# emreatilgan/P-Companion

Hardware: AMD Instinct MI355X
Metric: triplets/sec (Product2Vec pretrain step: gather+fwd+bwd+Adam) + P-Companion joint step under `joint` (higher is better)
Workload: dtype f32

## Files before the change

include/pcompanion_hip.h:

```cpp
#ifndef PCOMPANION_HIP_H
#define PCOMPANION_HIP_H

#include <stddef.h>
#include <stdint.h>

#ifdef __cplusplus
extern "C" {
#endif

#define PC_OK 0
#define PC_EINVAL (-1)
#define PC_ESHAPE (-2)
#define PC_EWORKSPACE (-3)
#define PC_EBATCHNORM (-4)
#define PC_ECOMM (-5)

#define PC_D 128
#define PC_H 256
#define PC_HEADS 4
#define PC_L 64
#define PC_MAX_SEG 4
#define PC_BN_SYNC_DOUBLES (PC_MAX_SEG * 2 * 256 + PC_MAX_SEG)

#define PC_ABI_VERSION 8
int pc_abi_version(void);
enum { PC_OPT_SIDE_QUEUE = 1, PC_OPT_SORTED_TABLE_GRADIENTS = 2, PC_OPT_BN_FINALIZE_SIDE = 3, PC_OPT_FUSED_LOSS = 4,
       PC_OPT_FUSED_OUT_CHAIN = 5 };
int pc_set_option(int option, int value);
int pc_get_option(int option, int* value);
int pc_release_device_state(void);
enum {
    PC_FLAG_EXP_NO_MFMA = 1, PC_FLAG_EXP_NO_SPLIT = 2, PC_FLAG_EXP_NO_LDSREAD = 4, PC_FLAG_EXP_NO_DMA = 8,
    PC_FLAG_EXP_NO_SLAB = 16, PC_FLAG_EXP_STAGGER = 32, PC_FLAG_EXP_DMA_L2 = 64, PC_FLAG_NT_TIMING = 128,
    PC_FLAG_JOINT_TIMING = 256, PC_FLAG_CHAIN_TIMING = 512, PC_FLAG_EXP_NO_BARRIER = 1024, PC_FLAG_EXP_NO_VMWAIT = 2048
};
unsigned pc_build_flags(void);

typedef struct {
    float p;
    uint64_t seed, offset;
} pc_dropout;

// ... 423 lines not shown
```

p_companion_amd/_lib.py:

```python
import ctypes
import os

_HERE = os.path.dirname(os.path.abspath(__file__))
LIB_PATH = os.path.join(_HERE, "libpcompanion_hip.so")
if os.environ.get("PC_DEV_LIB"):
    import sys as _sys
    LIB_PATH = os.path.abspath(os.environ["PC_DEV_LIB"])
    print(f"[p_companion_amd] PC_DEV_LIB: loading {LIB_PATH} instead of the in-tree library (developer A/B run)", file=_sys.stderr, flush=True)

c_f32p = ctypes.c_void_p
c_i32p = ctypes.c_void_p
PC_MAX_SEG = 4
D, H, HEADS, L = 128, 256, 4, 64

_ERR = {-1: "PC_EINVAL (null pointer / bad size)", -2: "PC_ESHAPE (unsupported dimension/alignment)",
        -3: "PC_EWORKSPACE (workspace too small)",
        -4: "PC_EBATCHNORM (a BatchNorm call group of one row in training mode)",
        -5: "PC_ECOMM (RCCL could not be loaded, or a communicator call failed)"}


class HipKernelError(RuntimeError):
    pass


# ... 33 lines not shown

_vp, _i, _sz, _f, _d, _u64, _i64 = (ctypes.c_void_p, ctypes.c_int, ctypes.c_size_t, ctypes.c_float,
                                    ctypes.c_double, ctypes.c_uint64, ctypes.c_int64)
_P = ctypes.POINTER

class AdamFused(ctypes.Structure):
    _fields_ = [("param", ctypes.c_void_p), ("grad", ctypes.c_void_p), ("exp_avg", ctypes.c_void_p), ("exp_avg_sq", ctypes.c_void_p),
                ("n", ctypes.c_size_t), ("step_count", ctypes.c_void_p), ("t", ctypes.c_int64),
                ("lr", ctypes.c_double), ("beta1", ctypes.c_double), ("beta2", ctypes.c_double), ("eps", ctypes.c_double)]


PC_OPT_SIDE_QUEUE = 1
PC_OPT_FUSED_OUT_CHAIN = 5
PC_OPT_FUSED_LOSS = 4
PC_OPT_BN_FINALIZE_SIDE = 3
PC_OPT_SORTED_TABLE_GRADIENTS = 2

SIGNATURES = {
    "pc_abi_version": (_i, []),
    "pc_build_flags": (ctypes.c_uint, []),
    "pc_set_option": (_i, [_i, _i]),
    "pc_get_option": (_i, [_i, ctypes.POINTER(ctypes.c_int)]),
    "pc_release_device_state": (_i, []),
    "pc_p2v_ffn_workspace_bytes": (_sz, [_i]),
    "pc_p2v_ffn_forward_train": (_i, [_P(P2VTensors), _vp, _vp, _i, _P(Segments), _i, _vp, _P(FfnSaved), _vp, _sz, _vp]),
    "pc_p2v_ffn_forward_eval": (_i, [_P(P2VTensors), _vp, _vp, _i, _vp, _vp, _sz, _vp]),
    "pc_p2v_ffn_backward": (_i, [_P(P2VTensors), _P(P2VTensors), _vp, _vp, _i, _P(Segments), _vp, _P(FfnSaved),
                                 _vp, _i, _vp, _sz, _vp]),
    "pc_p2v_attention_workspace_bytes": (_sz, [_i, _i]),
    "pc_p2v_attention_workspace_bytes_dim": (_sz, [_i, _i, _i]),
# ... 162 lines not shown
```

p_companion_amd/csrc/common.h:

```cpp
#pragma once
#include <hip/hip_runtime.h>
#include <stdint.h>
#include "../../include/pcompanion_hip.h"

typedef float f32x16 __attribute__((ext_vector_type(16)));
typedef float f32x4 __attribute__((ext_vector_type(4)));

#define PC_WAVE 64

#define PC_HIP_TRY(expr)                          \
    do {                                          \
        hipError_t _e = (expr);                   \
        if (_e != hipSuccess) return (int)_e;     \
    } while (0)

#define PC_TRY(expr)                 \
    do {                             \
        int _r = (expr);             \
        if (_r != 0) return _r;      \
    } while (0)

extern thread_local int pc_tls_launch_err;
#define PC_LAUNCH(...)                                                           \
    do {                                                                         \
// ... 425 lines not shown
struct TnArgs {
    const float* Z; int ldz;
    const float* A; int lda; const int32_t* gather;
    int R, No, Ni;
    SegInfo seg;
    int prologue; const float* pscale; const float* pshift;
    const float* zaux; int ldzaux;
    const float *z_mean, *z_invstd, *z_scale, *z_c1, *z_c2;
    const int32_t* z_onehot;
    float* dW; int lddw; float* db;
    int accumulate;
    float* slabs; size_t slab_floats;
};
struct TnDefer;
int launch_gemm_tn(const TnArgs& a, hipStream_t st, TnDefer* defer = nullptr);
int launch_gemm_tn_halves(const TnArgs& a, float* slabs0, float* slabs1, size_t slab_floats, hipStream_t st, TnDefer* defer);
size_t gemm_tn_workspace_floats(int R, int No, int Ni);
#define PC_TN_GROUP 10
#define PC_TN_EXTRA 2
#define PC_TN_RGROUP (PC_TN_GROUP + PC_TN_EXTRA + 4)
struct TnGroup { TnArgs a[PC_TN_GROUP]; int tiles_i[PC_TN_GROUP], nsplit[PC_TN_GROUP], rps[PC_TN_GROUP], block0[PC_TN_GROUP + 1], n; };
struct TnReduceJob { const float* slabs; int nsplit, n; float* out; int accumulate; };
#define PC_ADAM_REST (2 * (PC_TN_GROUP + PC_TN_EXTRA + 4) + 1)
struct AdamRider {
    float *p, *m, *v; const float* g; size_t n;
    int64_t* step_count; long long t; double lr, beta1, beta2; float omb1, beta2f, omb2, eps;
    int block0;
    int n_rest, rest_lo[PC_ADAM_REST], rest_hi[PC_ADAM_REST], rest_block0[PC_ADAM_REST + 1];
};
struct TnReduceGroup {
    const float* slabs[PC_TN_RGROUP]; float* dW[PC_TN_RGROUP]; float* db[PC_TN_RGROUP];
// ... 31 lines not shown
static inline void joint_fields(const pc_joint_tensors* t, float* (&out)[10]) {
    float* const f[10] = {t->itm_w, t->itm_b, t->typ_w, t->typ_b, t->dec_w, t->dec_b, t->enc_w, t->enc_b, t->comp_types, t->query_types};
    for (int i = 0; i < 10; i++) out[i] = f[i];
}
static inline bool joint_tensors_ok(const pc_joint_tensors* t, bool need_table) {
    if (!t || (need_table && !t->product_table)) return false;
    float* f[10];
    joint_fields(t, f);
    for (float* x : f)
        if (!x) return false;
    return true;
}

int pc_opt_sorted_tables();
int pc_opt_bn_finalize_side();
int pc_opt_fused_loss();
int pc_opt_fused_out_chain();
int triplet_loss_launch(const float* a, const float* p, const float* n, int batch, int k_neg, int dim, float margin,
                        float* loss, float* d_pos, float* d_neg, float* da, float* dp, float* dn, void* stream, int with_mean);
int launch_dropout(const float* x, size_t n, const pc_dropout& d, unsigned stream_id, float* y, hipStream_t st);
int launch_transpose(const float* in, int rows, int cols, float* out, hipStream_t st);
int ffn_forward_part1(const pc_p2v_tensors* p, const float* table, const int32_t* idx, int rows, const pc_segments* seg,
                      const pc_ffn_saved* sv, double* local_sums, void* ws, size_t ws_bytes, void* stream);
int ffn_forward_part2(const pc_p2v_tensors* p, int rows, const pc_segments* seg, int update_running, float* y,
                      const pc_ffn_saved* sv, const double* global_sums, void* ws, size_t ws_bytes, void* stream,
                      const TransposeBatch* ride = nullptr);
int ffn_backward_part1(const pc_p2v_tensors* p, const pc_p2v_tensors* g, const float* table, const int32_t* idx,
                       int rows, const pc_segments* seg, const float* dy, const pc_ffn_saved* sv, int with_dx,
                       int accumulate, double* local_sums, void* ws, size_t ws_bytes, void* stream, int transposed,
                       TnDefer* defer);
// ... 16 lines not shown
```

p_companion_amd/csrc/ffn.hip:

```cpp
#include "common.h"


#define BN_EPS 1e-5f
#define BN_MOMENTUM 0.1f

#define FIN_COLS 32
#define FIN_LANES 32
__device__ __forceinline__ void fold_partials(const float* p1, const float* p2, int t0, int t1, int j, int q,
                                              double (*red)[FIN_LANES][FIN_COLS], double* o1, double* o2) {
    double a = 0.0, b = 0.0, a1 = 0.0, b1 = 0.0;
    int t = t0 + q;
    for (; t + FIN_LANES < t1; t += 2 * FIN_LANES) {
        a += (double)p1[(size_t)t * PC_H + j];                b += (double)p2[(size_t)t * PC_H + j];
        a1 += (double)p1[(size_t)(t + FIN_LANES) * PC_H + j]; b1 += (double)p2[(size_t)(t + FIN_LANES) * PC_H + j];
    }
    if (t < t1) { a += (double)p1[(size_t)t * PC_H + j]; b += (double)p2[(size_t)t * PC_H + j]; }
    red[0][q][threadIdx.x] = a + a1;
    red[1][q][threadIdx.x] = b + b1;
    __syncthreads();
    if (q == 0) {
        double s1 = 0.0, s2 = 0.0;
#pragma unroll 8
        for (int i = 0; i < FIN_LANES; i++) { s1 += red[0][i][threadIdx.x]; s2 += red[1][i][threadIdx.x]; }
        *o1 = s1; *o2 = s2;
    }
    __syncthreads();
}

#define FIN4_CG 8
#define FIN4_LANES 64
#define FIN4_WAVES (FIN4_CG * FIN4_LANES / 64)
#define FIN4_BATCH 6
__device__ __forceinline__ void fold_partials_all4(const float* __restrict__ p1, const float* __restrict__ p2, const SegInfo& si,
                                                   int col0, double (*red)[2][PC_MAX_SEG][FIN_COLS], double* o1, double* o2) {
    const int cg = threadIdx.x, q = threadIdx.y;
    const int tid = q * FIN4_CG + cg, wave = tid >> 6, lane = tid & 63;
    double a[PC_MAX_SEG][4], b[PC_MAX_SEG][4];
#pragma unroll
    for (int s = 0; s < PC_MAX_SEG; s++)
#pragma unroll
        for (int c = 0; c < 4; c++) { a[s][c] = 0.0; b[s][c] = 0.0; }
    const int t_end = si.tile0[si.nseg];
    const int b1 = si.nseg > 1 ? si.tile0[1] : t_end, b2 = si.nseg > 2 ? si.tile0[2] : t_end, b3 = si.nseg > 3 ? si.tile0[3] : t_end;
    const size_t c0 = (size_t)col0 + cg * 4;
    for (int t = si.tile0[0] + q; t < t_end; t += FIN4_BATCH * FIN4_LANES) {
        float4 x[FIN4_BATCH], y[FIN4_BATCH];
#pragma unroll
        for (int u = 0; u < FIN4_BATCH; u++) {
            const int tt = t + u * FIN4_LANES;
            const int tc = tt < t_end ? tt : t;
            x[u] = *reinterpret_cast<const float4*>(p1 + (size_t)tc * PC_H + c0);
            y[u] = *reinterpret_cast<const float4*>(p2 + (size_t)tc * PC_H + c0);
        }
#pragma unroll
        for (int u = 0; u < FIN4_BATCH; u++) {
            const int tt = t + u * FIN4_LANES;
            const int sg = tt < t_end ? (tt >= b1) + (tt >= b2) + (tt >= b3) : -1;
#pragma unroll
            for (int s = 0; s < PC_MAX_SEG; s++) {
                const bool on = sg == s;
                a[s][0] += on ? (double)x[u].x : 0.0; a[s][1] += on ? (double)x[u].y : 0.0;
                a[s][2] += on ? (double)x[u].z : 0.0; a[s][3] += on ? (double)x[u].w : 0.0;
                b[s][0] += on ? (double)y[u].x : 0.0; b[s][1] += on ? (double)y[u].y : 0.0;
                b[s][2] += on ? (double)y[u].z : 0.0; b[s][3] += on ? (double)y[u].w : 0.0;
            }
        }
    }
#pragma unroll
    for (int s = 0; s < PC_MAX_SEG; s++)
#pragma unroll
        for (int c = 0; c < 4; c++) {
#pragma unroll
            for (int o = 8; o < 64; o <<= 1) { a[s][c] += __shfl_xor(a[s][c], o, 64); b[s][c] += __shfl_xor(b[s][c], o, 64); }
        }
    if (lane < FIN4_CG) {
#pragma unroll
        for (int s = 0; s < PC_MAX_SEG; s++)
#pragma unroll
            for (int c = 0; c < 4; c++) { red[wave][0][s][cg * 4 + c] = a[s][c]; red[wave][1][s][cg * 4 + c] = b[s][c]; }
    }
    __syncthreads();
    if (tid < PC_MAX_SEG * FIN_COLS) {
        const int s = tid / FIN_COLS, col = tid % FIN_COLS;
        double s1 = 0.0, s2 = 0.0;
#pragma unroll
        for (int w = 0; w < FIN4_WAVES; w++) { s1 += red[w][0][s][col]; s2 += red[w][1][s][col]; }
        *o1 = s1; *o2 = s2;
    }
}

__global__ __launch_bounds__(FIN_COLS * FIN_LANES) void bn_fold_kernel(const float* p1, const float* p2, SegInfo si,
                                                                       double* sums) {
    __shared__ double red[2][FIN_LANES][FIN_COLS];
    const int j = blockIdx.x * FIN_COLS + threadIdx.x, q = threadIdx.y;
    for (int s = 0; s < PC_MAX_SEG; s++) {
        double a = 0.0, b = 0.0;
        if (s < si.nseg) fold_partials(p1, p2, si.tile0[s], si.tile0[s + 1], j, q, red, &a, &b);
        if (q == 0) {
            sums[(2 * s) * PC_H + j] = a;
            sums[(2 * s + 1) * PC_H + j] = b;
            if (j == 0) sums[2 * PC_MAX_SEG * PC_H + s] = s < si.nseg ? (double)si.count[s] : 0.0;
        }
    }
// ... 2 lines not shown
__global__ __launch_bounds__(FIN4_CG * FIN4_LANES) void bn_finalize_fwd_kernel(
    const float* psum, const float* psq, SegInfo si, const double* gsum, const float* gamma, const float* beta,
    float* running_mean, float* running_var, int64_t* nbt, int update_running, float* mean_o, float* invstd_o,
    float* scale_o, float* shift_o, TransposeBatch ride, int tiles_x, int tiles_y) {
    __shared__ double red[FIN4_WAVES][2][PC_MAX_SEG][FIN_COLS];
    __shared__ float seg_mean[PC_MAX_SEG][FIN_COLS], seg_unb[PC_MAX_SEG][FIN_COLS];
    __shared__ int seg_live[PC_MAX_SEG][FIN_COLS];
    const int tid = threadIdx.y * FIN4_CG + threadIdx.x;
    if (blockIdx.x >= PC_H / FIN_COLS) {
        static_assert(sizeof(red) >= 32 * 33 * sizeof(float), "transpose tile");
        transpose_tile_body<FIN4_CG * FIN4_LANES>(ride, (int)blockIdx.x - PC_H / FIN_COLS, tiles_x, tiles_y,
                                                  reinterpret_cast<float(*)[33]>(&red[0][0][0][0]), tid);
        return;
    }
    double a = 0.0, b = 0.0;
    if (!gsum) fold_partials_all4(psum, psq, si, blockIdx.x * FIN_COLS, red, &a, &b);
    if (tid < PC_MAX_SEG * FIN_COLS) {
        const int s = tid / FIN_COLS, col = tid % FIN_COLS, j = blockIdx.x * FIN_COLS + col;
        double n = s < si.nseg ? (double)si.count[s] : 0.0;
        if (gsum && s < si.nseg) { a = gsum[(2 * s) * PC_H + j]; b = gsum[(2 * s + 1) * PC_H + j]; n = gsum[2 * PC_MAX_SEG * PC_H + s]; }
        int live = 0;
        if (s < si.nseg && n > 0) {
            const double m = a / n;
            double var = b / n - m * m;
            if (var < 0.0) var = 0.0;
            const float mf = (float)m, vf = (float)var;
            const float is = 1.0f / sqrtf(vf + BN_EPS);
            const float sc = gamma[j] * is;
            mean_o[s * PC_H + j] = mf;
            invstd_o[s * PC_H + j] = is;
            scale_o[s * PC_H + j] = sc;
// ... 21 lines not shown
    }
}

__global__ void bn_eval_coeff_kernel(const float* gamma, const float* beta, const float* running_mean,
                                     const float* running_var, float* scale_o, float* shift_o) {
    const int j = threadIdx.x;
    const float is = 1.0f / sqrtf(running_var[j] + BN_EPS);
    const float sc = gamma[j] * is;
    scale_o[j] = sc;
    shift_o[j] = beta[j] - running_mean[j] * sc;
}

__global__ __launch_bounds__(FIN4_CG * FIN4_LANES) void bn_finalize_bwd_kernel(
    const float* psum, const float* pdot, SegInfo si, const double* lsum, const double* gsum, const float* mean,
    const float* invstd, float* dgamma, float* dbeta, int accumulate, float* c1, float* c2) {
    __shared__ double red[FIN4_WAVES][2][PC_MAX_SEG][FIN_COLS];
    __shared__ double seg_g[PC_MAX_SEG][FIN_COLS], seg_b[PC_MAX_SEG][FIN_COLS];
    const int tid = threadIdx.y * FIN4_CG + threadIdx.x;
    double a = 0.0, b = 0.0;
    if (!lsum) fold_partials_all4(psum, pdot, si, blockIdx.x * FIN_COLS, red, &a, &b);
    if (tid < PC_MAX_SEG * FIN_COLS) {
        const int s = tid / FIN_COLS, col = tid % FIN_COLS, j = blockIdx.x * FIN_COLS + col;
        double tg = 0.0, tb = 0.0;
        if (s < si.nseg) {
            double n = si.count[s];
            if (lsum) { a = lsum[(2 * s) * PC_H + j]; b = lsum[(2 * s + 1) * PC_H + j]; }
            const double is = (double)invstd[s * PC_H + j], mu = (double)mean[s * PC_H + j];
            b = is * (b - mu * a);
            tb = a;
            tg = b;
            double ga = a, gb = b;
            if (gsum) {
                ga = gsum[(2 * s) * PC_H + j];
                gb = is * (gsum[(2 * s + 1) * PC_H + j] - mu * ga);
                n = gsum[2 * PC_MAX_SEG * PC_H + s];
            }
            c1[s * PC_H + j] = n > 0 ? (float)(ga / n) : 0.f;
            c2[s * PC_H + j] = n > 0 ? (float)(gb / n) : 0.f;
        }
        seg_g[s][col] = tg;
        seg_b[s][col] = tb;
    }
    __syncthreads();
    if (tid < FIN_COLS) {
        const int j = blockIdx.x * FIN_COLS + tid;
        double tg = 0.0, tb = 0.0;
        for (int s = 0; s < si.nseg; s++) { tg += seg_g[s][tid]; tb += seg_b[s][tid]; }
        dgamma[j] = accumulate ? dgamma[j] + (float)tg : (float)tg;
        dbeta[j] = accumulate ? dbeta[j] + (float)tb : (float)tb;
    }
}

__global__ void bn_bwd_apply_kernel(float* dz, const float* h0, int rows, SegInfo si, const float* mean,
                                    const float* invstd, const float* scale, const float* c1, const float* c2) {
    const int c4 = (threadIdx.x & 63) * 4;
    const int rl = threadIdx.x >> 6;
    for (int r = blockIdx.x * 4 + rl; r < rows; r += gridDim.x * 4) {
        const int s = seg_of_row(si, r);
        const float m = row_multiplicity(si, r);
        float4 g = *reinterpret_cast<float4*>(dz + (size_t)r * PC_H + c4);
        const float4 h = *reinterpret_cast<const float4*>(h0 + (size_t)r * PC_H + c4);
        const float4 mu = *reinterpret_cast<const float4*>(mean + s * PC_H + c4);
        const float4 is = *reinterpret_cast<const float4*>(invstd + s * PC_H + c4);
        const float4 sc = *reinterpret_cast<const float4*>(scale + s * PC_H + c4);
        const float4 a = *reinterpret_cast<const float4*>(c1 + s * PC_H + c4);
// ... 226 lines not shown
    TnArgs t5 = {};
    t5.Z = dy; t5.ldz = D; t5.A = sv->a2; t5.lda = PC_H; t5.R = rows; t5.No = D; t5.Ni = PC_H; t5.seg = si;
    t5.dW = g->w5; t5.lddw = PC_H; t5.db = g->b5; t5.accumulate = accumulate; t5.slabs = w.slabs[0];
    t5.slab_floats = w.slab_floats;
    if (D == 256 && rows >= 8192 && (size_t)2 * 128 * ((size_t)128 * PC_H + 128) <= w.slab_floats) {
        const size_t half = (size_t)128 * ((size_t)128 * PC_H + 128);
        PC_TRY(launch_gemm_tn_halves(t5, w.slabs[0], w.slabs[0] + half, half, st, df));
    } else {
        PC_TRY(launch_gemm_tn(t5, st, df));
    }

    NtArgs b2 = nt_plain(w.dz2, PC_H, w.w3t, PC_H, nullptr, w.dz1, PC_H, rows, PC_H, PC_H, si);
    b2.epilogue = NT_EPI_DTANH_BN; b2.aux = sv->h0; b2.ldaux = PC_H; b2.escale = sv->bn_scale; b2.eshift = sv->bn_shift;
    b2.stats = NT_STAT_BNBWD; b2.stat_sum = w.stat_a; b2.stat_aux = w.stat_b;
    PC_TRY(launch_gemm_nt(b2, st));
    if (df->fork && !local_sums) {
        if (pc_opt_bn_finalize_side()) {
            PC_TRY(pc_fork_begin(df->fork, 1, st));
            PC_LAUNCH(bn_finalize_bwd_kernel, dim3(PC_H / FIN_COLS), dim3(FIN4_CG, FIN4_LANES), 0, df->fork->side, w.stat_a, w.stat_b, si,
                      nullptr, nullptr, sv->bn_mean, sv->bn_invstd, g->gamma, g->beta, accumulate, w.c1, w.c2);
            PC_TRY(pc_launch_status());
            df->bn_finalized = 1;
        } else {
            PC_LAUNCH(bn_finalize_bwd_kernel, dim3(PC_H / FIN_COLS), dim3(FIN4_CG, FIN4_LANES), 0, st, w.stat_a, w.stat_b, si,
                      nullptr, nullptr, sv->bn_mean, sv->bn_invstd, g->gamma, g->beta, accumulate, w.c1, w.c2);
            PC_TRY(pc_launch_status());
            df->bn_finalized = 2;
        }
    }

    TnArgs t3 = {};
    t3.Z = w.dz2; t3.ldz = PC_H; t3.A = sv->a1 ? sv->a1 : sv->h0; t3.lda = PC_H; t3.R = rows; t3.No = PC_H; t3.Ni = PC_H; t3.seg = si;
    if (!sv->a1) { t3.prologue = NT_PRO_BNTANH; t3.pscale = sv->bn_scale; t3.pshift = sv->bn_shift; }
    t3.dW = g->w3; t3.lddw = PC_H; t3.db = g->b3; t3.accumulate = accumulate; t3.slabs = w.slabs[1];
    t3.slab_floats = w.slab_floats;
    if (sv->a1) {
        if (rows >= 8192 && (size_t)128 * ((size_t)128 * PC_H + 128) <= w.slab_floats) {
            PC_TRY(launch_gemm_tn_halves(t3, w.slabs[1], w.slabs[2], w.slab_floats, st, df));
        } else {
            for (int half = 0; half < 2; half++) {
                TnArgs th = t3;
                th.Z = w.dz2 + half * (PC_H / 2); th.No = PC_H / 2;
                th.dW = g->w3 + (size_t)half * (PC_H / 2) * PC_H; th.db = g->b3 + half * (PC_H / 2);
                th.slabs = w.slabs[1 + half];
                PC_TRY(launch_gemm_tn(th, st, df));
            }
        }
    } else {
        PC_TRY(launch_gemm_tn(t3, st, df));
    }
    if (local_sums) {
        PC_LAUNCH(bn_fold_kernel, dim3(PC_H / FIN_COLS), dim3(FIN_COLS, FIN_LANES), 0, st, w.stat_a, w.stat_b, si, local_sums);
        PC_TRY(pc_launch_status());
// ... 57 lines not shown
```

p_companion_amd/csrc/gemm_tn.hip:

```cpp
#include <atomic>
#include <mutex>
#include "common.h"

#define TM 128
#define TK 32

__device__ __forceinline__ void tn_small_body(const TnArgs& a, int tiles_i, int nsplit, int rows_per_split, int bid) {
    __shared__ __attribute__((aligned(16))) float smem[2][2][TK * TM];

    const int tid = threadIdx.x, lane = tid & 63, w = tid >> 6, wo = w >> 1, wi = w & 1;
    const int split = bid % nsplit;
    const int tile = bid / nsplit;
    const int o0 = (tile / tiles_i) * TM, i0 = (tile % tiles_i) * TM;
    const int r_begin = split * rows_per_split;
    const int r_end = min(a.R, r_begin + rows_per_split);

    const int lrow = tid >> 5, lcol = (tid & 31) * 4;
    const bool zcol_ok = o0 + lcol < a.No, acol_ok = i0 + lcol < a.Ni;

    float4 rz[4], ra[4];
    float4 dbacc = make_float4(0.f, 0.f, 0.f, 0.f);
    int zseg = -1;
    float4 zmu, zis, zsc, zc1, zc2;
    auto gload = [&](int r0) {
// ... 126 lines not shown

typedef __attribute__((address_space(3))) void* tn_lptr_t;
__device__ __attribute__((aligned(64))) float pc_tn_zero_chunk[16];
#pragma clang diagnostic push
#pragma clang diagnostic ignored "-Winline-asm"
__device__ __forceinline__ void tn_dma16(const float* gsrc, unsigned lds_addr) {
    asm volatile("s_mov_b32 m0, %1\n\ts_nop 0\n\tglobal_load_lds_dwordx4 %0, off" ::"v"(gsrc), "s"(lds_addr) : "memory", "m0");
}
#pragma clang diagnostic pop
__device__ __forceinline__ void tn_lds_sync() {
    asm volatile("s_waitcnt lgkmcnt(0)" ::: "memory");
    __builtin_amdgcn_s_barrier();
    asm volatile("" ::: "memory");
}

template <int WO, int WI, int TO, int TI, int TKC, int NST, bool APRO, bool ZPRO>
__global__ __launch_bounds__(64 * WO * WI, WO * WI / 4) void gemm_tn8_kernel(TnArgs a, int nsplit, int rows_per_split, int halves,
                                                                             size_t slab_half_off) {
    constexpr int NWV = WO * WI, THREADS = 64 * NWV;
    constexpr int NO = WO * TO * 32, NI = WI * TI * 32;
    constexpr int ZRS = NO == 256 ? 260 : NO, ARS = NI == 256 ? 260 : NI;
    constexpr bool ZSW = NO == 128, ASW = NI == 128;
    static_assert((NO == 128 || NO == 256) && (NI == 128 || NI == 256), "image widths");
    constexpr int ZF = TKC * ZRS, AF = TKC * ARS;
    constexpr int STAGE = ZF * (ZPRO ? 2 : 1) + AF;
    constexpr int JZ = TKC * NO / 256 / NWV, JA = TKC * NI / 256 / NWV;
    static_assert((TKC * NO) % (256 * NWV) == 0 && (TKC * NI) % (256 * NWV) == 0, "images must split into whole wave instructions over the waves");
    constexpr int JALL = JZ * (ZPRO ? 2 : 1) + JA;
    __shared__ __attribute__((aligned(1024))) float smem[NST * STAGE];

    const int tid = threadIdx.x, lane = tid & 63;
    const int w = __builtin_amdgcn_readfirstlane(tid >> 6), wo = w % WO, wi = w / WO;
    const int half = halves == 2 ? ((int)blockIdx.x >> 3) & 1 : 0;
    const int split = halves == 2 ? (((int)blockIdx.x >> 4) << 3) + ((int)blockIdx.x & 7) : (int)blockIdx.x;
    if (halves == 2) {
        a.Z += half * (WO * TO * 32);
        a.slabs += half * slab_half_off;
        if (a.db) a.db += half * (WO * TO * 32);
    }
    const int r_begin = split * rows_per_split;
    const int r_end = min(a.R, r_begin + rows_per_split);
    const float* const zsrc0 = pc_tn_zero_chunk;
    const unsigned lds0 = (unsigned)(uintptr_t)(tn_lptr_t)&smem[0];

    int zr[JZ], zc[JZ], ar[JA], ac[JA];
    unsigned zd[JZ], ad[JA];
#pragma unroll
    for (int j = 0; j < JZ; j++) {
        const int g = w + NWV * j, f = g * 256 + lane * 4;
        zr[j] = f / NO; zc[j] = f % NO;
        if (ZSW && (zr[j] & 8)) zc[j] ^= 32;
        zd[j] = (NO == 256 ? g * ZRS : g * 256) * 4;
    }
#pragma unroll
    for (int j = 0; j < JA; j++) {
        const int g = w + NWV * j, f = g * 256 + lane * 4;
        ar[j] = f / NI; ac[j] = f % NI;
        if (ASW && (ar[j] & 8)) ac[j] ^= 32;
// ... 325 lines not shown

int launch_gemm_tn(const TnArgs& a, hipStream_t st, TnDefer* defer) {
    if ((!a.Z && !a.z_onehot) || !a.A || !a.dW || !a.slabs || a.R <= 0 || a.No <= 0 || a.Ni <= 0) return PC_EINVAL;
    if (a.No % 4 || a.Ni % 4 || (a.Z && a.ldz % 4) || a.lda % 4 || a.lddw != a.Ni) return PC_ESHAPE;
    if (a.z_onehot && (a.zaux || tn_full_tile(a.R, a.No, a.Ni))) return PC_ESHAPE;
    if (((uintptr_t)a.dW & 15) || (a.db && ((uintptr_t)a.db & 15)) || ((uintptr_t)a.slabs & 15)) return PC_ESHAPE;
    int nsplit, rps;
    tn_plan(a.R, a.No, a.Ni, &nsplit, &rps);
    if ((size_t)nsplit * ((size_t)a.No * a.Ni + a.No) > a.slab_floats) return PC_EWORKSPACE;
    const int tiles_o = (a.No + TM - 1) / TM, tiles_i = (a.Ni + TM - 1) / TM;
    const bool apro = a.prologue == NT_PRO_BNTANH, zpro = a.zaux != nullptr;
    const int pb = pc_prof_begin(PC_KIND_GEMM_TN, 2.0 * a.R * (double)a.No * a.Ni, st);
    if (tn_full_tile(a.R, a.No, a.Ni) && !(apro && zpro)) {
#define TN8(WO, WI, TO, TI, TKC, NST)                                                                         \
    do {                                                                                                      \
        if (apro) PC_LAUNCH((gemm_tn8_kernel<WO, WI, TO, TI, TKC, NST, true, false>), dim3(nsplit), dim3(64 * WO * WI), 0, st, a, nsplit, rps, 1, (size_t)0);    \
        else if (zpro && a.Ni > 128) PC_LAUNCH((gemm_tn8_kernel<2, 4, 4, 2, 16, 3, false, true>), dim3(nsplit), dim3(512), 0, st, a, nsplit, rps, 1, (size_t)0);  \
        else if (zpro) PC_LAUNCH((gemm_tn8_kernel<4, 2, 2, 2, 16, 3, false, true>), dim3(nsplit), dim3(512), 0, st, a, nsplit, rps, 1, (size_t)0);  \
        else PC_LAUNCH((gemm_tn8_kernel<WO, WI, TO, TI, TKC, NST, false, false>), dim3(nsplit), dim3(64 * WO * WI), 0, st, a, nsplit, rps, 1, (size_t)0);        \
    } while (0)
        if (a.No > 128 && a.Ni > 128) TN8(2, 4, 4, 2, 16, 3);
        else if (a.No > 128) TN8(4, 2, 2, 2, 32, 2);
        else TN8(2, 4, 2, 2, 32, 2);
#undef TN8
    } else {
        PC_LAUNCH(gemm_tn_kernel, dim3(tiles_o * tiles_i * nsplit), dim3(256), 0, st, a, tiles_i, nsplit, rps);
    }
    pc_prof_end(pb, st);
    PC_TRY(pc_launch_status());
    const int n_w = a.No * a.Ni, n_b = a.No;
    const int threads = (n_w + (a.db ? n_b : 0)) / 4 * 8;
    if (defer) return tn_defer_push(defer, a.slabs, a.slab_floats, nsplit, n_w, n_b, a.dW, a.db, a.accumulate);
    PC_LAUNCH(tn_reduce_kernel, dim3((threads + 255) / 256), dim3(256), 0, st, a.slabs, nsplit, n_w, n_b,
                       a.dW, a.db, a.accumulate);
    return pc_launch_status();
}

int launch_gemm_tn_halves(const TnArgs& a, float* slabs0, float* slabs1, size_t slab_floats, hipStream_t st, TnDefer* defer) {
    if (!a.Z || !a.A || !a.dW || !slabs0 || !slabs1 || !defer || a.R <= 0) return PC_EINVAL;
    if (a.No != 256 || a.Ni != 256 || a.ldz % 4 || a.lda % 4 || a.lddw != a.Ni || a.prologue != NT_PRO_NONE || a.zaux || a.z_onehot || a.gather)
        return PC_ESHAPE;
    if (slabs1 < slabs0) return PC_EINVAL;
    const int nsplit = 128;
    int rps = (a.R + nsplit - 1) / nsplit;
    rps = (rps + 31) / 32 * 32;
    const int used = (a.R + rps - 1) / rps;
    const size_t per = (size_t)128 * a.Ni + 128;
    if ((size_t)nsplit * per > slab_floats) return PC_EWORKSPACE;
    (void)used;
    TnArgs h = a;
    h.No = 128; h.slabs = slabs0; h.slab_floats = slab_floats;
    const int pb = pc_prof_begin(PC_KIND_GEMM_TN, 2.0 * a.R * (double)a.No * a.Ni, st);
    PC_LAUNCH((gemm_tn8_kernel<2, 4, 2, 2, 32, 2, false, false>), dim3(2 * nsplit), dim3(512), 0, st, h, nsplit, rps, 2,
              (size_t)(slabs1 - slabs0));
    pc_prof_end(pb, st);
    PC_TRY(pc_launch_status());
    PC_TRY(tn_defer_push(defer, slabs0, slab_floats, nsplit, 128 * a.Ni, 128, a.dW, a.db, a.accumulate));
    return tn_defer_push(defer, slabs1, slab_floats, nsplit, 128 * a.Ni, 128, a.dW + (size_t)128 * a.Ni, a.db ? a.db + 128 : nullptr,
                         a.accumulate);
}

namespace {
struct ForkSlot { int dev; hipStream_t main_st; int state; PcFork f; };
ForkSlot g_fork_slots[32];
std::mutex g_fork_mu;
std::atomic<int> g_opt_side_queue{1};
std::atomic<int> g_opt_sorted_tables{1};
std::atomic<int> g_opt_bn_finalize_side{0};
std::atomic<int> g_opt_fused_loss{1};
std::atomic<int> g_opt_fused_out_chain{1};
std::atomic<int>* opt_slot(int option) {
    switch (option) {
        case PC_OPT_SIDE_QUEUE: return &g_opt_side_queue;
        case PC_OPT_SORTED_TABLE_GRADIENTS: return &g_opt_sorted_tables;
        case PC_OPT_BN_FINALIZE_SIDE: return &g_opt_bn_finalize_side;
        case PC_OPT_FUSED_LOSS: return &g_opt_fused_loss;
        case PC_OPT_FUSED_OUT_CHAIN: return &g_opt_fused_out_chain;
        default: return nullptr;
    }
}
}
int pc_opt_sorted_tables() { return g_opt_sorted_tables.load(std::memory_order_relaxed); }
int pc_opt_bn_finalize_side() { return g_opt_bn_finalize_side.load(std::memory_order_relaxed); }
int pc_opt_fused_loss() { return g_opt_fused_loss.load(std::memory_order_relaxed); }
int pc_opt_fused_out_chain() { return g_opt_fused_out_chain.load(std::memory_order_relaxed); }

extern "C" int pc_set_option(int option, int value) {
    std::atomic<int>* o = opt_slot(option);
    if (!o || (value != 0 && value != 1)) return PC_EINVAL;
    o->store(value, std::memory_order_relaxed);
    return PC_OK;
}
extern "C" int pc_get_option(int option, int* value) {
    std::atomic<int>* o = opt_slot(option);
    if (!o || !value) return PC_EINVAL;
    *value = o->load(std::memory_order_relaxed);
    return PC_OK;
}
// ... 193 lines not shown
```

Baseline: 5.144 million.

## Fold BatchNorm backward finalize into idle blocks of the halves TN GEMM launch

Result: faster. 5.211 million (median of 6 runs) (+1.3%).

```diff
diff --git a/include/pcompanion_hip.h b/include/pcompanion_hip.h
--- a/include/pcompanion_hip.h
+++ b/include/pcompanion_hip.h
@@ -25,7 +25,7 @@
 #define PC_ABI_VERSION 8
 int pc_abi_version(void);
 enum { PC_OPT_SIDE_QUEUE = 1, PC_OPT_SORTED_TABLE_GRADIENTS = 2, PC_OPT_BN_FINALIZE_SIDE = 3, PC_OPT_FUSED_LOSS = 4,
-       PC_OPT_FUSED_OUT_CHAIN = 5 };
+       PC_OPT_FUSED_OUT_CHAIN = 5, PC_OPT_BN_FINALIZE_RIDES = 6 };
 int pc_set_option(int option, int value);
 int pc_get_option(int option, int* value);
 int pc_release_device_state(void);
diff --git a/p_companion_amd/_lib.py b/p_companion_amd/_lib.py
--- a/p_companion_amd/_lib.py
+++ b/p_companion_amd/_lib.py
@@ -71,6 +71,7 @@
 PC_OPT_FUSED_OUT_CHAIN = 5
 PC_OPT_FUSED_LOSS = 4
 PC_OPT_BN_FINALIZE_SIDE = 3
+PC_OPT_BN_FINALIZE_RIDES = 6
 PC_OPT_SORTED_TABLE_GRADIENTS = 2
 
 SIGNATURES = {
diff --git a/p_companion_amd/csrc/bn_finalize.h b/p_companion_amd/csrc/bn_finalize.h
--- /dev/null
+++ b/p_companion_amd/csrc/bn_finalize.h
@@ -0,0 +1,116 @@
+#pragma once
+#include "common.h"
+
+#define FIN_COLS 32
+
+#ifdef __HIPCC__
+#define FIN4_CG 8
+#define FIN4_LANES 64
+#define FIN4_WAVES (FIN4_CG * FIN4_LANES / 64)
+#define FIN4_BATCH 6
+__device__ __forceinline__ void fold_partials_all4(const float* __restrict__ p1, const float* __restrict__ p2, const SegInfo& si,
+                                                   int col0, int tid, double (*red)[2][PC_MAX_SEG][FIN_COLS], double* o1, double* o2) {
+    const int cg = tid % FIN4_CG, q = tid / FIN4_CG;
+    const int wave = tid >> 6, lane = tid & 63;
+    double a[PC_MAX_SEG][4], b[PC_MAX_SEG][4];
+#pragma unroll
+    for (int s = 0; s < PC_MAX_SEG; s++)
+#pragma unroll
+        for (int c = 0; c < 4; c++) { a[s][c] = 0.0; b[s][c] = 0.0; }
+    const int t_end = si.tile0[si.nseg];
+    const int b1 = si.nseg > 1 ? si.tile0[1] : t_end, b2 = si.nseg > 2 ? si.tile0[2] : t_end, b3 = si.nseg > 3 ? si.tile0[3] : t_end;
+    const size_t c0 = (size_t)col0 + cg * 4;
+    for (int t = si.tile0[0] + q; t < t_end; t += FIN4_BATCH * FIN4_LANES) {
+        float4 x[FIN4_BATCH], y[FIN4_BATCH];
+#pragma unroll
+        for (int u = 0; u < FIN4_BATCH; u++) {
+            const int tt = t + u * FIN4_LANES;
+            const int tc = tt < t_end ? tt : t;
+            x[u] = *reinterpret_cast<const float4*>(p1 + (size_t)tc * PC_H + c0);
+            y[u] = *reinterpret_cast<const float4*>(p2 + (size_t)tc * PC_H + c0);
+        }
+#pragma unroll
+        for (int u = 0; u < FIN4_BATCH; u++) {
+            const int tt = t + u * FIN4_LANES;
+            const int sg = tt < t_end ? (tt >= b1) + (tt >= b2) + (tt >= b3) : -1;
+#pragma unroll
+            for (int s = 0; s < PC_MAX_SEG; s++) {
+                const bool on = sg == s;
+                a[s][0] += on ? (double)x[u].x : 0.0; a[s][1] += on ? (double)x[u].y : 0.0;
+                a[s][2] += on ? (double)x[u].z : 0.0; a[s][3] += on ? (double)x[u].w : 0.0;
+                b[s][0] += on ? (double)y[u].x : 0.0; b[s][1] += on ? (double)y[u].y : 0.0;
+                b[s][2] += on ? (double)y[u].z : 0.0; b[s][3] += on ? (double)y[u].w : 0.0;
+            }
+        }
+    }
+#pragma unroll
+    for (int s = 0; s < PC_MAX_SEG; s++)
+#pragma unroll
+        for (int c = 0; c < 4; c++) {
+#pragma unroll
+            for (int o = 8; o < 64; o <<= 1) { a[s][c] += __shfl_xor(a[s][c], o, 64); b[s][c] += __shfl_xor(b[s][c], o, 64); }
+        }
+    if (lane < FIN4_CG) {
+#pragma unroll
+        for (int s = 0; s < PC_MAX_SEG; s++)
+#pragma unroll
+            for (int c = 0; c < 4; c++) { red[wave][0][s][cg * 4 + c] = a[s][c]; red[wave][1][s][cg * 4 + c] = b[s][c]; }
+    }
+    __syncthreads();
+    if (tid < PC_MAX_SEG * FIN_COLS) {
+        const int s = tid / FIN_COLS, col = tid % FIN_COLS;
+        double s1 = 0.0, s2 = 0.0;
+#pragma unroll
+        for (int w = 0; w < FIN4_WAVES; w++) { s1 += red[w][0][s][col]; s2 += red[w][1][s][col]; }
+        *o1 = s1; *o2 = s2;
+    }
+}
+#endif
+
+struct BnFinBwd {
+    const float *psum, *pdot; const double *lsum, *gsum; const float *mean, *invstd;
+    float *dgamma, *dbeta; int accumulate; float *c1, *c2;
+};
+struct BnFinBwdScratch {
+    double red[FIN4_WAVES][2][PC_MAX_SEG][FIN_COLS];
+    double seg_g[PC_MAX_SEG][FIN_COLS], seg_b[PC_MAX_SEG][FIN_COLS];
+};
+#ifdef __HIPCC__
+__device__ __forceinline__ void bn_finalize_bwd_body(const BnFinBwd& f, const SegInfo& si, int cb, int tid, BnFinBwdScratch* sm) {
+    double a = 0.0, b = 0.0;
+    if (!f.lsum) fold_partials_all4(f.psum, f.pdot, si, cb * FIN_COLS, tid, sm->red, &a, &b);
+    if (tid < PC_MAX_SEG * FIN_COLS) {
+        const int s = tid / FIN_COLS, col = tid % FIN_COLS, j = cb * FIN_COLS + col;
+        double tg = 0.0, tb = 0.0;
+        if (s < si.nseg) {
+            double n = si.count[s];
+            if (f.lsum) { a = f.lsum[(2 * s) * PC_H + j]; b = f.lsum[(2 * s + 1) * PC_H + j]; }
+            const double is = (double)f.invstd[s * PC_H + j], mu = (double)f.mean[s * PC_H + j];
+            b = is * (b - mu * a);
+            tb = a;
+            tg = b;
+            double ga = a, gb = b;
+            if (f.gsum) {
+                ga = f.gsum[(2 * s) * PC_H + j];
+                gb = is * (f.gsum[(2 * s + 1) * PC_H + j] - mu * ga);
+                n = f.gsum[2 * PC_MAX_SEG * PC_H + s];
+            }
+            f.c1[s * PC_H + j] = n > 0 ? (float)(ga / n) : 0.f;
+            f.c2[s * PC_H + j] = n > 0 ? (float)(gb / n) : 0.f;
+        }
+        sm->seg_g[s][col] = tg;
+        sm->seg_b[s][col] = tb;
+    }
+    __syncthreads();
+    if (tid < FIN_COLS) {
+        const int j = cb * FIN_COLS + tid;
+        double tg = 0.0, tb = 0.0;
+        for (int s = 0; s < si.nseg; s++) { tg += sm->seg_g[s][tid]; tb += sm->seg_b[s][tid]; }
+        f.dgamma[j] = f.accumulate ? f.dgamma[j] + (float)tg : (float)tg;
+        f.dbeta[j] = f.accumulate ? f.dbeta[j] + (float)tb : (float)tb;
+    }
+}
+#endif
+
+#define PC_TN_RIDERS (PC_H / FIN_COLS)
+struct TnRider { int n; int block[PC_TN_RIDERS]; BnFinBwd fin; SegInfo si; };
diff --git a/p_companion_amd/csrc/common.h b/p_companion_amd/csrc/common.h
--- a/p_companion_amd/csrc/common.h
+++ b/p_companion_amd/csrc/common.h
@@ -463,7 +463,9 @@
 };
 struct TnDefer;
 int launch_gemm_tn(const TnArgs& a, hipStream_t st, TnDefer* defer = nullptr);
-int launch_gemm_tn_halves(const TnArgs& a, float* slabs0, float* slabs1, size_t slab_floats, hipStream_t st, TnDefer* defer);
+struct TnRider;
+int launch_gemm_tn_halves(const TnArgs& a, float* slabs0, float* slabs1, size_t slab_floats, hipStream_t st, TnDefer* defer,
+                          const TnRider* rider = nullptr);
 size_t gemm_tn_workspace_floats(int R, int No, int Ni);
 #define PC_TN_GROUP 10
 #define PC_TN_EXTRA 2
@@ -525,6 +527,7 @@
 
 int pc_opt_sorted_tables();
 int pc_opt_bn_finalize_side();
+int pc_opt_bn_finalize_rides();
 int pc_opt_fused_loss();
 int pc_opt_fused_out_chain();
 int triplet_loss_launch(const float* a, const float* p, const float* n, int batch, int k_neg, int dim, float margin,
diff --git a/p_companion_amd/csrc/ffn.hip b/p_companion_amd/csrc/ffn.hip
--- a/p_companion_amd/csrc/ffn.hip
+++ b/p_companion_amd/csrc/ffn.hip
@@ -1,10 +1,9 @@
 #include "common.h"
-
+#include "bn_finalize.h"
 
 #define BN_EPS 1e-5f
 #define BN_MOMENTUM 0.1f
 
-#define FIN_COLS 32
 #define FIN_LANES 32
 __device__ __forceinline__ void fold_partials(const float* p1, const float* p2, int t0, int t1, int j, int q,
                                               double (*red)[FIN_LANES][FIN_COLS], double* o1, double* o2) {
@@ -25,68 +24,6 @@
         *o1 = s1; *o2 = s2;
     }
     __syncthreads();
-}
-
-#define FIN4_CG 8
-#define FIN4_LANES 64
-#define FIN4_WAVES (FIN4_CG * FIN4_LANES / 64)
-#define FIN4_BATCH 6
-__device__ __forceinline__ void fold_partials_all4(const float* __restrict__ p1, const float* __restrict__ p2, const SegInfo& si,
-                                                   int col0, double (*red)[2][PC_MAX_SEG][FIN_COLS], double* o1, double* o2) {
-    const int cg = threadIdx.x, q = threadIdx.y;
-    const int tid = q * FIN4_CG + cg, wave = tid >> 6, lane = tid & 63;
-    double a[PC_MAX_SEG][4], b[PC_MAX_SEG][4];
-#pragma unroll
-    for (int s = 0; s < PC_MAX_SEG; s++)
-#pragma unroll
-        for (int c = 0; c < 4; c++) { a[s][c] = 0.0; b[s][c] = 0.0; }
-    const int t_end = si.tile0[si.nseg];
-    const int b1 = si.nseg > 1 ? si.tile0[1] : t_end, b2 = si.nseg > 2 ? si.tile0[2] : t_end, b3 = si.nseg > 3 ? si.tile0[3] : t_end;
-    const size_t c0 = (size_t)col0 + cg * 4;
-    for (int t = si.tile0[0] + q; t < t_end; t += FIN4_BATCH * FIN4_LANES) {
-        float4 x[FIN4_BATCH], y[FIN4_BATCH];
-#pragma unroll
-        for (int u = 0; u < FIN4_BATCH; u++) {
-            const int tt = t + u * FIN4_LANES;
-            const int tc = tt < t_end ? tt : t;
-            x[u] = *reinterpret_cast<const float4*>(p1 + (size_t)tc * PC_H + c0);
-            y[u] = *reinterpret_cast<const float4*>(p2 + (size_t)tc * PC_H + c0);
-        }
-#pragma unroll
-        for (int u = 0; u < FIN4_BATCH; u++) {
-            const int tt = t + u * FIN4_LANES;
-            const int sg = tt < t_end ? (tt >= b1) + (tt >= b2) + (tt >= b3) : -1;
-#pragma unroll
-            for (int s = 0; s < PC_MAX_SEG; s++) {
-                const bool on = sg == s;
-                a[s][0] += on ? (double)x[u].x : 0.0; a[s][1] += on ? (double)x[u].y : 0.0;
-                a[s][2] += on ? (double)x[u].z : 0.0; a[s][3] += on ? (double)x[u].w : 0.0;
-                b[s][0] += on ? (double)y[u].x : 0.0; b[s][1] += on ? (double)y[u].y : 0.0;
-                b[s][2] += on ? (double)y[u].z : 0.0; b[s][3] += on ? (double)y[u].w : 0.0;
-            }
-        }
-    }
-#pragma unroll
-    for (int s = 0; s < PC_MAX_SEG; s++)
-#pragma unroll
-        for (int c = 0; c < 4; c++) {
-#pragma unroll
-            for (int o = 8; o < 64; o <<= 1) { a[s][c] += __shfl_xor(a[s][c], o, 64); b[s][c] += __shfl_xor(b[s][c], o, 64); }
-        }
-    if (lane < FIN4_CG) {
-#pragma unroll
-        for (int s = 0; s < PC_MAX_SEG; s++)
-#pragma unroll
-            for (int c = 0; c < 4; c++) { red[wave][0][s][cg * 4 + c] = a[s][c]; red[wave][1][s][cg * 4 + c] = b[s][c]; }
-    }
-    __syncthreads();
-    if (tid < PC_MAX_SEG * FIN_COLS) {
-        const int s = tid / FIN_COLS, col = tid % FIN_COLS;
-        double s1 = 0.0, s2 = 0.0;
-#pragma unroll
-        for (int w = 0; w < FIN4_WAVES; w++) { s1 += red[w][0][s][col]; s2 += red[w][1][s][col]; }
-        *o1 = s1; *o2 = s2;
-    }
 }
 
 __global__ __launch_bounds__(FIN_COLS * FIN_LANES) void bn_fold_kernel(const float* p1, const float* p2, SegInfo si,
@@ -119,7 +56,7 @@
         return;
     }
     double a = 0.0, b = 0.0;
-    if (!gsum) fold_partials_all4(psum, psq, si, blockIdx.x * FIN_COLS, red, &a, &b);
+    if (!gsum) fold_partials_all4(psum, psq, si, blockIdx.x * FIN_COLS, tid, red, &a, &b);
     if (tid < PC_MAX_SEG * FIN_COLS) {
         const int s = tid / FIN_COLS, col = tid % FIN_COLS, j = blockIdx.x * FIN_COLS + col;
         double n = s < si.nseg ? (double)si.count[s] : 0.0;
@@ -171,41 +108,9 @@
 __global__ __launch_bounds__(FIN4_CG * FIN4_LANES) void bn_finalize_bwd_kernel(
     const float* psum, const float* pdot, SegInfo si, const double* lsum, const double* gsum, const float* mean,
     const float* invstd, float* dgamma, float* dbeta, int accumulate, float* c1, float* c2) {
-    __shared__ double red[FIN4_WAVES][2][PC_MAX_SEG][FIN_COLS];
-    __shared__ double seg_g[PC_MAX_SEG][FIN_COLS], seg_b[PC_MAX_SEG][FIN_COLS];
-    const int tid = threadIdx.y * FIN4_CG + threadIdx.x;
-    double a = 0.0, b = 0.0;
-    if (!lsum) fold_partials_all4(psum, pdot, si, blockIdx.x * FIN_COLS, red, &a, &b);
-    if (tid < PC_MAX_SEG * FIN_COLS) {
-        const int s = tid / FIN_COLS, col = tid % FIN_COLS, j = blockIdx.x * FIN_COLS + col;
-        double tg = 0.0, tb = 0.0;
-        if (s < si.nseg) {
-            double n = si.count[s];
-            if (lsum) { a = lsum[(2 * s) * PC_H + j]; b = lsum[(2 * s + 1) * PC_H + j]; }
-            const double is = (double)invstd[s * PC_H + j], mu = (double)mean[s * PC_H + j];
-            b = is * (b - mu * a);
-            tb = a;
-            tg = b;
-            double ga = a, gb = b;
-            if (gsum) {
-                ga = gsum[(2 * s) * PC_H + j];
-                gb = is * (gsum[(2 * s + 1) * PC_H + j] - mu * ga);
-                n = gsum[2 * PC_MAX_SEG * PC_H + s];
-            }
-            c1[s * PC_H + j] = n > 0 ? (float)(ga / n) : 0.f;
-            c2[s * PC_H + j] = n > 0 ? (float)(gb / n) : 0.f;
-        }
-        seg_g[s][col] = tg;
-        seg_b[s][col] = tb;
-    }
-    __syncthreads();
-    if (tid < FIN_COLS) {
-        const int j = blockIdx.x * FIN_COLS + tid;
-        double tg = 0.0, tb = 0.0;
-        for (int s = 0; s < si.nseg; s++) { tg += seg_g[s][tid]; tb += seg_b[s][tid]; }
-        dgamma[j] = accumulate ? dgamma[j] + (float)tg : (float)tg;
-        dbeta[j] = accumulate ? dbeta[j] + (float)tb : (float)tb;
-    }
+    __shared__ BnFinBwdScratch sm;
+    const BnFinBwd f = {psum, pdot, lsum, gsum, mean, invstd, dgamma, dbeta, accumulate, c1, c2};
+    bn_finalize_bwd_body(f, si, (int)blockIdx.x, (int)(threadIdx.y * FIN4_CG + threadIdx.x), &sm);
 }
 
 __global__ void bn_bwd_apply_kernel(float* dz, const float* h0, int rows, SegInfo si, const float* mean,
@@ -462,13 +367,20 @@
     b2.epilogue = NT_EPI_DTANH_BN; b2.aux = sv->h0; b2.ldaux = PC_H; b2.escale = sv->bn_scale; b2.eshift = sv->bn_shift;
     b2.stats = NT_STAT_BNBWD; b2.stat_sum = w.stat_a; b2.stat_aux = w.stat_b;
     PC_TRY(launch_gemm_nt(b2, st));
+    TnRider fin_rider = {};
     if (df->fork && !local_sums) {
+        const BnFinBwd fin = {w.stat_a, w.stat_b, nullptr, nullptr, sv->bn_mean, sv->bn_invstd, g->gamma, g->beta, accumulate, w.c1, w.c2};
         if (pc_opt_bn_finalize_side()) {
             PC_TRY(pc_fork_begin(df->fork, 1, st));
             PC_LAUNCH(bn_finalize_bwd_kernel, dim3(PC_H / FIN_COLS), dim3(FIN4_CG, FIN4_LANES), 0, df->fork->side, w.stat_a, w.stat_b, si,
                       nullptr, nullptr, sv->bn_mean, sv->bn_invstd, g->gamma, g->beta, accumulate, w.c1, w.c2);
             PC_TRY(pc_launch_status());
             df->bn_finalized = 1;
+        } else if (pc_opt_bn_finalize_rides() && sv->a1 && rows >= 8192 && (size_t)128 * ((size_t)128 * PC_H + 128) <= w.slab_floats) {
+            fin_rider.n = PC_TN_RIDERS;
+            fin_rider.fin = fin;
+            fin_rider.si = si;
+            df->bn_finalized = 2;
         } else {
             PC_LAUNCH(bn_finalize_bwd_kernel, dim3(PC_H / FIN_COLS), dim3(FIN4_CG, FIN4_LANES), 0, st, w.stat_a, w.stat_b, si,
                       nullptr, nullptr, sv->bn_mean, sv->bn_invstd, g->gamma, g->beta, accumulate, w.c1, w.c2);
@@ -484,7 +396,7 @@
     t3.slab_floats = w.slab_floats;
     if (sv->a1) {
         if (rows >= 8192 && (size_t)128 * ((size_t)128 * PC_H + 128) <= w.slab_floats) {
-            PC_TRY(launch_gemm_tn_halves(t3, w.slabs[1], w.slabs[2], w.slab_floats, st, df));
+            PC_TRY(launch_gemm_tn_halves(t3, w.slabs[1], w.slabs[2], w.slab_floats, st, df, fin_rider.n ? &fin_rider : nullptr));
         } else {
             for (int half = 0; half < 2; half++) {
                 TnArgs th = t3;
diff --git a/p_companion_amd/csrc/gemm_tn.hip b/p_companion_amd/csrc/gemm_tn.hip
--- a/p_companion_amd/csrc/gemm_tn.hip
+++ b/p_companion_amd/csrc/gemm_tn.hip
@@ -1,6 +1,8 @@
 #include <atomic>
 #include <mutex>
+#include <type_traits>
 #include "common.h"
+#include "bn_finalize.h"
 
 #define TM 128
 #define TK 32
@@ -164,9 +166,11 @@
     asm volatile("" ::: "memory");
 }
 
-template <int WO, int WI, int TO, int TI, int TKC, int NST, bool APRO, bool ZPRO>
+struct TnNoRider {};
+template <int WO, int WI, int TO, int TI, int TKC, int NST, bool APRO, bool ZPRO, bool RIDER = false>
 __global__ __launch_bounds__(64 * WO * WI, WO * WI / 4) void gemm_tn8_kernel(TnArgs a, int nsplit, int rows_per_split, int halves,
-                                                                             size_t slab_half_off) {
+                                                                             size_t slab_half_off,
+                                                                             std::conditional_t<RIDER, TnRider, TnNoRider> rider) {
     constexpr int NWV = WO * WI, THREADS = 64 * NWV;
     constexpr int NO = WO * TO * 32, NI = WI * TI * 32;
     constexpr int ZRS = NO == 256 ? 260 : NO, ARS = NI == 256 ? 260 : NI;
@@ -192,6 +196,16 @@
     const int r_end = min(a.R, r_begin + rows_per_split);
     const float* const zsrc0 = pc_tn_zero_chunk;
     const unsigned lds0 = (unsigned)(uintptr_t)(tn_lptr_t)&smem[0];
+    if constexpr (RIDER) {
+        int rid = -1;
+#pragma unroll
+        for (int i = 0; i < PC_TN_RIDERS; i++) rid = (int)blockIdx.x == rider.block[i] ? i : rid;
+        if (rid >= 0) {
+            static_assert(sizeof(smem) >= sizeof(BnFinBwdScratch) && THREADS == FIN4_CG * FIN4_LANES, "a finalize workgroup");
+            bn_finalize_bwd_body(rider.fin, rider.si, rid, (int)threadIdx.x, reinterpret_cast<BnFinBwdScratch*>(smem));
+            return;
+        }
+    }
 
     int zr[JZ], zc[JZ], ar[JA], ac[JA];
     unsigned zd[JZ], ad[JA];
@@ -547,10 +561,10 @@
     if (tn_full_tile(a.R, a.No, a.Ni) && !(apro && zpro)) {
 #define TN8(WO, WI, TO, TI, TKC, NST)                                                                         \
     do {                                                                                                      \
-        if (apro) PC_LAUNCH((gemm_tn8_kernel<WO, WI, TO, TI, TKC, NST, true, false>), dim3(nsplit), dim3(64 * WO * WI), 0, st, a, nsplit, rps, 1, (size_t)0);    \
-        else if (zpro && a.Ni > 128) PC_LAUNCH((gemm_tn8_kernel<2, 4, 4, 2, 16, 3, false, true>), dim3(nsplit), dim3(512), 0, st, a, nsplit, rps, 1, (size_t)0);  \
-        else if (zpro) PC_LAUNCH((gemm_tn8_kernel<4, 2, 2, 2, 16, 3, false, true>), dim3(nsplit), dim3(512), 0, st, a, nsplit, rps, 1, (size_t)0);  \
-        else PC_LAUNCH((gemm_tn8_kernel<WO, WI, TO, TI, TKC, NST, false, false>), dim3(nsplit), dim3(64 * WO * WI), 0, st, a, nsplit, rps, 1, (size_t)0);        \
+        if (apro) PC_LAUNCH((gemm_tn8_kernel<WO, WI, TO, TI, TKC, NST, true, false>), dim3(nsplit), dim3(64 * WO * WI), 0, st, a, nsplit, rps, 1, (size_t)0, TnNoRider{});    \
+        else if (zpro && a.Ni > 128) PC_LAUNCH((gemm_tn8_kernel<2, 4, 4, 2, 16, 3, false, true>), dim3(nsplit), dim3(512), 0, st, a, nsplit, rps, 1, (size_t)0, TnNoRider{});  \
+        else if (zpro) PC_LAUNCH((gemm_tn8_kernel<4, 2, 2, 2, 16, 3, false, true>), dim3(nsplit), dim3(512), 0, st, a, nsplit, rps, 1, (size_t)0, TnNoRider{});  \
+        else PC_LAUNCH((gemm_tn8_kernel<WO, WI, TO, TI, TKC, NST, false, false>), dim3(nsplit), dim3(64 * WO * WI), 0, st, a, nsplit, rps, 1, (size_t)0, TnNoRider{});        \
     } while (0)
         if (a.No > 128 && a.Ni > 128) TN8(2, 4, 4, 2, 16, 3);
         else if (a.No > 128) TN8(4, 2, 2, 2, 32, 2);
@@ -569,7 +583,8 @@
     return pc_launch_status();
 }
 
-int launch_gemm_tn_halves(const TnArgs& a, float* slabs0, float* slabs1, size_t slab_floats, hipStream_t st, TnDefer* defer) {
+int launch_gemm_tn_halves(const TnArgs& a, float* slabs0, float* slabs1, size_t slab_floats, hipStream_t st, TnDefer* defer,
+                          const TnRider* rider) {
     if (!a.Z || !a.A || !a.dW || !slabs0 || !slabs1 || !defer || a.R <= 0) return PC_EINVAL;
     if (a.No != 256 || a.Ni != 256 || a.ldz % 4 || a.lda % 4 || a.lddw != a.Ni || a.prologue != NT_PRO_NONE || a.zaux || a.z_onehot || a.gather)
         return PC_ESHAPE;
@@ -580,16 +595,33 @@
     const int used = (a.R + rps - 1) / rps;
     const size_t per = (size_t)128 * a.Ni + 128;
     if ((size_t)nsplit * per > slab_floats) return PC_EWORKSPACE;
-    (void)used;
     TnArgs h = a;
     h.No = 128; h.slabs = slabs0; h.slab_floats = slab_floats;
+    TnRider rd = {};
+    int blocks = 2 * nsplit, nred = nsplit;
+    if (rider && rider->n) {
+        if (rider->n != PC_TN_RIDERS) return PC_EINVAL;
+        rd = *rider;
+        int k = 0;
+        for (int b = 0; b < 2 * nsplit && k < rd.n; b++)
+            if (((b >> 4) << 3) + (b & 7) >= used) rd.block[k++] = b;
+        if (k == rd.n) nred = used;
+        else {
+            for (k = 0; k < rd.n; k++) rd.block[k] = blocks + k;
+            blocks += rd.n;
+        }
+    }
     const int pb = pc_prof_begin(PC_KIND_GEMM_TN, 2.0 * a.R * (double)a.No * a.Ni, st);
-    PC_LAUNCH((gemm_tn8_kernel<2, 4, 2, 2, 32, 2, false, false>), dim3(2 * nsplit), dim3(512), 0, st, h, nsplit, rps, 2,
-              (size_t)(slabs1 - slabs0));
+    if (rd.n)
+        PC_LAUNCH((gemm_tn8_kernel<2, 4, 2, 2, 32, 2, false, false, true>), dim3(blocks), dim3(512), 0, st, h, nsplit, rps, 2,
+                  (size_t)(slabs1 - slabs0), rd);
+    else
+        PC_LAUNCH((gemm_tn8_kernel<2, 4, 2, 2, 32, 2, false, false>), dim3(blocks), dim3(512), 0, st, h, nsplit, rps, 2,
+                  (size_t)(slabs1 - slabs0), TnNoRider{});
     pc_prof_end(pb, st);
     PC_TRY(pc_launch_status());
-    PC_TRY(tn_defer_push(defer, slabs0, slab_floats, nsplit, 128 * a.Ni, 128, a.dW, a.db, a.accumulate));
-    return tn_defer_push(defer, slabs1, slab_floats, nsplit, 128 * a.Ni, 128, a.dW + (size_t)128 * a.Ni, a.db ? a.db + 128 : nullptr,
+    PC_TRY(tn_defer_push(defer, slabs0, slab_floats, nred, 128 * a.Ni, 128, a.dW, a.db, a.accumulate));
+    return tn_defer_push(defer, slabs1, slab_floats, nred, 128 * a.Ni, 128, a.dW + (size_t)128 * a.Ni, a.db ? a.db + 128 : nullptr,
                          a.accumulate);
 }
 
@@ -600,6 +632,7 @@
 std::atomic<int> g_opt_side_queue{1};
 std::atomic<int> g_opt_sorted_tables{1};
 std::atomic<int> g_opt_bn_finalize_side{0};
+std::atomic<int> g_opt_bn_finalize_rides{1};
 std::atomic<int> g_opt_fused_loss{1};
 std::atomic<int> g_opt_fused_out_chain{1};
 std::atomic<int>* opt_slot(int option) {
@@ -609,12 +642,14 @@
         case PC_OPT_BN_FINALIZE_SIDE: return &g_opt_bn_finalize_side;
         case PC_OPT_FUSED_LOSS: return &g_opt_fused_loss;
         case PC_OPT_FUSED_OUT_CHAIN: return &g_opt_fused_out_chain;
+        case PC_OPT_BN_FINALIZE_RIDES: return &g_opt_bn_finalize_rides;
         default: return nullptr;
     }
 }
 }
 int pc_opt_sorted_tables() { return g_opt_sorted_tables.load(std::memory_order_relaxed); }
 int pc_opt_bn_finalize_side() { return g_opt_bn_finalize_side.load(std::memory_order_relaxed); }
+int pc_opt_bn_finalize_rides() { return g_opt_bn_finalize_rides.load(std::memory_order_relaxed); }
 int pc_opt_fused_loss() { return g_opt_fused_loss.load(std::memory_order_relaxed); }
 int pc_opt_fused_out_chain() { return g_opt_fused_out_chain.load(std::memory_order_relaxed); }
 
```
